# AlexanderDzhoganov/sphereflake-raytracer

Hardware: AMD Instinct MI355X
Metric: Mrays/sec into G-buffer at 1920x1080 depth-8; frame time ms (higher is better)
Workload: dtype f32

## Files before the change

### __graft_entry__.py

```python
import os
import subprocess
import sys

REPO = os.path.dirname(os.path.abspath(__file__))
PKG = os.path.join(REPO, "sphereflake-raytracer_amd")


def _paths():
    for p in (REPO, PKG):
        if p not in sys.path:
            sys.path.insert(0, p)


def build() -> None:
    _paths()
    jobs = str(min(16, os.cpu_count() or 1))
    subprocess.check_call(["make", "-s", "-j", jobs, "-C", PKG, "all"])
    subprocess.check_call(["make", "-s", "-C", PKG, "testlibs"])
    subprocess.check_call(["make", "-s", "-C", os.path.join(REPO, "oracle"), "all"])
    if os.path.isdir("/root/reference/sphereflake"):
        subprocess.check_call(["make", "-s", "-C", os.path.join(REPO, "oracle"), "ref"])
    import sphereflake_amd
    sphereflake_amd.lib()


def smoke() -> None:
    _paths()
    import numpy as np
    import sphereflake_amd as sf
    from oracle import pyoracle
    if not os.path.exists(sf.LIB_PATH):
        sf.build()
    W, H, K = 96, 64, 0.25
    with sf.Sphereflake(W, H, device=0) as s:
        cam = sf.config_camera(W, H, K)
        s.SetCamera(cam)
        s.Render(emit_aux=True)
        pos, nrm, mint, idx = s.download(aux=True)
        st = s.stats()
    o, tl, tr, bl = cam.corners()
    setup = {"W": W, "H": H, "origin": o, "tl": tl, "tr": tr, "bl": bl,
             "root": sf.root_transform(o), "children": sf.child_transforms()}
    ref = pyoracle.render(setup)
    for k, got in (("pos4", pos), ("nrm4", nrm), ("minT", mint), ("index", idx)):
        if not np.array_equal(np.ascontiguousarray(ref[k]).view(np.uint8), np.ascontiguousarray(got).view(np.uint8)):
            raise AssertionError(f"smoke: {k} differs from the oracle")
    if st.max_depth != ref["stats"]["max_depth"]:
        raise AssertionError("smoke: max depth differs from the oracle")
    print(f"smoke ok: {W}x{H} K={K} max_depth={st.max_depth} hits={ref['stats']['hits']}")


if __name__ == "__main__":
    build()
    if len(sys.argv) > 1 and sys.argv[1] == "smoke":
        smoke()
```

### sphereflake-raytracer_amd/csrc/sf_internal.h

```cpp
#pragma once

#include <stdint.h>

#if defined(__HIPCC__) || defined(__HIP__)
#define SF_HD __host__ __device__
#else
#define SF_HD
#endif

#define SF_DEPTH_TABLE 33
#ifndef SF_OCCL_MARGIN
#define SF_OCCL_MARGIN 0x1.8p-9f
#endif
#define SF_TILE 8
#define SF_WAVES_PER_BLOCK 4
#ifndef SF_WAVES_PER_EU
#define SF_WAVES_PER_EU 8
#endif
#ifndef SF_PAIR_WAVES_PER_EU
#define SF_PAIR_WAVES_PER_EU 7
#endif
#ifndef SF_TRACE_WAVES
#define SF_TRACE_WAVES 1
#endif
#define SF_LDS_ROOT 16
#define SF_LDS_CONE 8
#define SF_LDS_PLANE 38
#define SF_LDS_COLS 27
#define SF_LDS_TABLE (SF_LDS_PLANE + 3 * SF_LDS_COLS)
#define SF_LDS_E 32
#define SF_LDS_LEVEL (SF_LDS_TABLE + SF_LDS_E + 1)
#define SF_LDS_WAVE_FLOATS(levels) (SF_LDS_ROOT + SF_LDS_CONE + ((levels) - 1) * SF_LDS_LEVEL)
#define SF_RAYS_CSTACK (3 * 64)
#define SF_LDS_RAYS_FLOATS(levels) (SF_LDS_WAVE_FLOATS((levels) + 1) + (levels) * SF_RAYS_CSTACK)

#define SF_QUEUES 32u
#define SF_QUEUE_STRIDE 32u
#define SF_QUEUE_WORD(parity, k) (SF_QUEUE_STRIDE + ((parity) * SF_QUEUES + (k)) * SF_QUEUE_STRIDE)
#define SF_COUNTER_WORDS (SF_QUEUE_STRIDE + 2u * SF_QUEUES * SF_QUEUE_STRIDE)

#define SF_DIAG_SLOTS 16
#define SF_DIAG_WAVES 65536u
#define SF_TRACE_WORDS(ntiles) ((size_t)(ntiles) * 15u + SF_DIAG_SLOTS + 2u * SF_DIAG_WAVES)

#define SF_FLAG_NO_LOD_CULL 1u
#define SF_FLAG_NO_CONE_CULL 2u
#define SF_FLAG_DIAG_HALF 4u
#define SF_FLAG_DIAG_HALF_SEL 8u
#define SF_FLAG_DIAG_UNITS 0x20u
#define SF_FLAG_DIAG_NO_OWNER 0x40u
#define SF_FLAG_PRIO_FLAT 0x80u
#define SF_FLAG_NO_OCCL_CULL 0x100u
#define SF_FLAG_NO_DEPTH_SEED 0x10u
#define SF_FLAG_NO_FRONT_FIRST 0x200u
#define SF_FLAG_DIAG_FORCE_RETRACE 0x400u
#define SF_FLAG_TIE_INLINE 0x800u
#define SF_FLAG_REDO_PASS 0x1000u
#define SF_FLAG_SUBTREE 0x2000u
#define SF_FLAG_HALVES 0x4000u
#define SF_FLAG_FORCE_MIXED 0x8000u

struct DepthTables {
    float r2_bound[SF_DEPTH_TABLE];
    float r2_self[SF_DEPTH_TABLE];
    float scale[SF_DEPTH_TABLE];
    float lod[SF_DEPTH_TABLE];
};

struct DeviceConsts {
    float child[9][16];
    DepthTables dt;
    float depth8[SF_DEPTH_TABLE][8];
    uint32_t lut[2048];
    uint32_t sobol[2][52];
    float rw, rh;
    uint32_t fast_div, tx_magic;
};

struct PacketLane {
    float px, py, pz, nx, ny, nz, min_t;
    uint32_t pixel;
};

struct FrameArgs {
    uint32_t W, H;
    float fw, fh;
    float o[3], tl[3], dh[3], dv[3];
    float root[12];
    uint32_t tiles_x;
    uint32_t tile_rows;
    uint32_t tiles_per_band;
    uint32_t band_count, band_index;
    uint32_t compact;
    uint32_t packed;
    uint32_t max_depth;
    uint32_t emit_aux;
    uint32_t flags;
    const DeviceConsts* consts;
    float* pos;
    float* nrm;
    float* min_t;
    uint32_t* hit_index;
    int32_t* stats;
    uint64_t* tile_trace;
    uint64_t* phase_sums;
    uint32_t* counters;
    uint32_t* overflow_list;
    uint32_t parity;
    uint32_t* tile_cost;
    const uint32_t* tile_order;
    const uint32_t* order_meta;
    uint32_t* chunk_cnt;
    uint32_t* part_cost;
// ... 126 lines not shown
```

### sphereflake-raytracer_amd/csrc/sf_kernels.hip

```cpp
#include <hip/hip_runtime.h>
#include <float.h>
#include <stddef.h>
#include <stdint.h>

#include "sf_internal.h"

#pragma clang fp contract(off)

#define SF_MAX_LEVELS 31

namespace {

__device__ __forceinline__ float rsqrtps_x86(float x, const uint32_t* __restrict__ lut)
{
    const uint32_t b = __float_as_uint(x);
    const uint32_t E = (b >> 23) & 0xffu;
    const uint32_t key = ((E & 1u) << 10) | ((b & 0x7fffffu) >> 13);
    const int32_t E0 = (E & 1u) ? 127 : 128;
    const int32_t k = ((int32_t)E - E0) / 2;
    uint32_t r = (uint32_t)((int32_t)lut[key] - k * (1 << 23));
    if ((b & 0x7fffffffu) > 0x7f800000u) r = b | 0x00400000u;
    else if (E == 0u) r = (b & 0x80000000u) | 0x7f800000u;
    else if (b & 0x80000000u) r = 0xffc00000u;
    else if (E == 0xffu) r = 0u;
// ... 195 lines not shown
{
    __builtin_amdgcn_wave_barrier();
    __asm__ volatile("" ::: "memory");
}

__device__ __forceinline__ float readlane_f(float v, uint32_t l)
{
    return __int_as_float(__builtin_amdgcn_readlane(__float_as_int(v), (int)l));
}
__device__ __forceinline__ uint32_t writelane_u(uint32_t v, uint32_t l, uint32_t old)
{
    return (threadIdx.x & 63u) == l ? v : old;
}

__device__ int sf_amdgcn_writelane(int v, int l, int old) __asm("llvm.amdgcn.writelane.i32");
__device__ __forceinline__ uint32_t writelane_s(uint32_t v, uint32_t l, uint32_t old)
{
    return (uint32_t)sf_amdgcn_writelane((int)v, (int)l, (int)old);
}

__device__ __forceinline__ void wave_atomic_add_u64(uint64_t* p, uint64_t v)
{
    uint64_t saved;
    const uint32_t zero = 0u;
    __asm__ volatile(
        "s_mov_b64 %0, exec\n\t"
        "s_mov_b64 exec, 1\n\t"
        "global_atomic_add_x2 %1, %2, %3\n\t"
        "s_waitcnt vmcnt(0)\n\t"
        "s_mov_b64 exec, %0\n\t"
        : "=&s"(saved)
        : "v"(zero), "v"(v), "s"(p)
        : "memory");
}

#ifdef SF_PHASE_STAMPS
#define SF_STAMP_DECL uint64_t ph_last = __builtin_amdgcn_s_memtime(), ph_sum[7] = {0, 0, 0, 0, 0, 0, 0}
#define SF_STAMP(k)                                                                            \
    do {                                                                                       \
        uint64_t t_;                                                                           \
        __builtin_amdgcn_sched_barrier(0);                                                     \
        __asm__ volatile("s_memtime %0\n\ts_waitcnt lgkmcnt(0)" : "=s"(t_)::"memory");         \
        __builtin_amdgcn_sched_barrier(0);                                                     \
        ph_sum[k] += t_ - ph_last;                                                             \
        ph_last = t_;                                                                          \
    } while (0)
#define SF_STAMP_FLUSH(p)                                                                      \
    do {                                                                                       \
        if (p) {                                                                               \
            for (int k_ = 0; k_ < 7; ++k_) wave_atomic_add_u64((uint64_t*)(p) + k_, ph_sum[k_]);  \
        }                                                                                      \
    } while (0)
#elif defined(SF_COUNTS)
#define SF_STAMP_DECL uint64_t ph_sum[16] = {0, 0, 0, 0, 0, 0, 0, 0, 0, 0, 0, 0, 0, 0, 0, 0}
#define SF_STAMP(k)
#define SF_COUNT(k, v) (ph_sum[k] += (v))
#define SF_STAMP_FLUSH(p)                                                                      \
    do {                                                                                       \
        if (p) {                                                                               \
            ph_sum[15] = 1;                                                                    \
            for (int k_ = 0; k_ < 16; ++k_) wave_atomic_add_u64((uint64_t*)(p) + k_, ph_sum[k_]); \
        }                                                                                      \
    } while (0)
#else
#define SF_STAMP_DECL
#define SF_STAMP(k)
#define SF_STAMP_FLUSH(p) (void)(p)
#endif
#ifndef SF_COUNT
#define SF_COUNT(k, v)
#endif

__device__ __forceinline__ float4 depth_consts(const DeviceConsts* K, uint32_t d)
{
#if defined(__HIP_DEVICE_COMPILE__)
    typedef const __attribute__((address_space(4))) float4* ConstF4;
    typedef const __attribute__((address_space(4))) char* ConstC;
    return *(ConstF4)((ConstC)(const void*)K->depth8 + (d << 5));
#else
    return reinterpret_cast<const float4*>(K->depth8)[2u * d];
#endif
}
__device__ __forceinline__ float4 depth_consts_at(const DeviceConsts* K, uint32_t o)
{
#if defined(__HIP_DEVICE_COMPILE__)
    typedef const __attribute__((address_space(4))) float4* ConstF4;
    typedef const __attribute__((address_space(4))) char* ConstC;
    return *(ConstF4)((ConstC)(const void*)K->depth8 + o);
#else
    return reinterpret_cast<const float4*>(K->depth8)[o >> 4];
#endif
}
__device__ __forceinline__ float depth_word_at(const DeviceConsts* K, uint32_t o, uint32_t w)
{
#if defined(__HIP_DEVICE_COMPILE__)
    typedef const __attribute__((address_space(4))) float* ConstF;
    typedef const __attribute__((address_space(4))) char* ConstC;
    return *(ConstF)((ConstC)(const void*)K->depth8 + o + 4u * w);
#else
    return reinterpret_cast<const float*>(K->depth8)[(o >> 2) + w];
#endif
}
__device__ __forceinline__ float depth_leaf(const DeviceConsts* K, uint32_t d)
{
#if defined(__HIP_DEVICE_COMPILE__)
    typedef const __attribute__((address_space(4))) float* ConstF;
    typedef const __attribute__((address_space(4))) char* ConstC;
    return *(ConstF)((ConstC)(const void*)K->depth8 + (d << 5) + 16u);
#else
    return reinterpret_cast<const float4*>(K->depth8)[2u * d + 1u].x;
#endif
}

#define SF_STATUS_OVERFLOW 1u
// ... 80 lines not shown
}
template <class S2m>
__device__ __forceinline__ void stage_cone(const TraverseLds& L, uint32_t lane, bool cone_cull, float ax, float ay,
                                           float az, S2m s2m)
{
    float cosT = 0.0f, sinT = 1.0f;
    if (cone_cull) {
        const float sm = __builtin_amdgcn_sqrtf(wave_max_pos(s2m())) * (1.0f + 0x1p-16f) + 0x1p-16f;
        if (sm < 0.5f) {
            sinT = sm;
            cosT = __builtin_amdgcn_sqrtf(1.0f - sm * sm) * (1.0f - 0x1p-16f);
        }
    }
    if (lane < 5u) L.cone()[lane] = lane == 0u ? ax : lane == 1u ? ay : lane == 2u ? az : lane == 3u ? cosT : sinT;
}

__device__ __forceinline__ uint64_t lod_expands(float tca, float d2, float xs, bool hb, uint64_t hbm, float R2b, float T,
                                                float Tfar)
{
    const uint64_t nearm = wave_ballot(tca < T);
    const uint64_t farm = wave_ballot(tca * (1.0f - 0x1p-8f) >= Tfar);
    if ((hbm & ~(nearm | farm)) == 0ull) return hbm & nearm;
    const float sq = __builtin_amdgcn_sqrtf(xs);
    const float s_lo = __uint_as_float((uint32_t)max((int32_t)__float_as_uint(sq) - 2, 0));
    const float s_hi = __uint_as_float(__float_as_uint(sq) + 2u);
    const float t_hi = tca - s_lo;
    const float t_lo = tca - s_hi;
    const uint64_t tinym = wave_ballot(xs < 0x1p-96f);
    const float thx = sel_mask(t_hi, __builtin_inff(), tinym);
    const float tlx = sel_mask(t_lo, -__builtin_inff(), tinym);
    const float th = hb ? thx : __builtin_inff();
    const float tl = hb ? tlx : __builtin_inff();
    uint64_t exm = wave_ballot(th < T);
    const uint64_t undm = wave_ballot(sel_mask(tl, __builtin_inff(), exm) < T);
    if (undm) {
        const float te = near_root_exact(tca, d2, R2b);
        exm |= undm & wave_ballot(te < T);
    }
    return exm;
}

__device__ __forceinline__ bool child_expands(float cx, float cy, float cz, float cc, float dx, float dy, float dz,
                                              float actv, float R2b, float T, float Tfar)
{
    const float tca = (cx * dx + cy * dy) + cz * dz;
    const float d2 = cc - tca * tca;
    const float xs = R2b - d2;
    const bool hb = __builtin_fminf(__builtin_fminf(tca, xs), actv) >= 0.0f;
    const uint64_t hbm = wave_ballot(hb);
    return hbm != 0ull && lod_expands(tca, d2, xs, hb, hbm, R2b, T, Tfar) != 0ull;
}

template <bool ANYHIT, bool INDEX_ORDER = false>
__device__ __forceinline__ uint64_t accept_self(HitState& h, uint64_t& ancm, uint32_t& status, bool flag_ties,
                                                const float4 pc, float tca, float d2, uint32_t dd, float actv,
                                                uint32_t idx, float R2s)
{
    const uint64_t hsm = wave_ballot(__builtin_fminf(__builtin_fminf(tca, R2s - d2), actv) >= 0.0f);
    if (hsm) {
        const float xs = R2s - d2;
        float ts;
        if ((wave_ballot(!(xs >= 0x1p-96f)) & hsm) != 0ull) ts = near_root_exact(tca, d2, R2s);
        else ts = near_root_big(tca, xs);
        uint64_t accm = hsm & wave_ballot(ts < h.minT);
        if constexpr (ANYHIT) {
            uint32_t hd = (uint32_t)h.depth;
            sel_in_place(hd, dd, accm);
            h.depth = (int32_t)hd;
            return accm;
        }
        const uint64_t tie = hsm & wave_ballot(ts == h.minT);
        if constexpr (INDEX_ORDER) accm |= tie & ancm;
        else if (tie != 0ull) {
            accm |= tie & ancm;
            if (flag_ties && (tie & ~ancm) != 0ull) status |= SF_STATUS_TIE;
        }
        sel_in_place(h.minT, ts, accm);
        sel_in_place(h.cx, pc.x, accm);
        sel_in_place(h.cy, pc.y, accm);
        sel_in_place(h.cz, pc.z, accm);
        sel_in_place(h.index, idx, accm);
        uint32_t hd = (uint32_t)h.depth;
        sel_in_place(hd, dd, accm);
        h.depth = (int32_t)hd;
        ancm |= accm;
        return accm;
    }
    return 0ull;
}

template <bool ANYHIT>
__device__ __forceinline__ uint64_t occluded(float tca, float minT, float cull_t, float cull_r)
{
    float v = tca - minT;
    if constexpr (!ANYHIT) v = __builtin_fminf(v, tca - cull_t);
    return wave_ballot(v - SF_OCCL_MARGIN * tca > cull_r);
}

struct ChildBuild {
    float x, y, z, w;
    uint32_t M, front;
    float4 dtc;
};
__device__ __forceinline__ ChildBuild build_children(const DeviceConsts* K, const TraverseLds& L, const BuildLane& B,
                                                     const float4 pc, const float* col, uint32_t cs, uint32_t ko,
                                                     float kp, uint32_t index_order)
{
    lds_fence();
    const float3 p0 = *reinterpret_cast<const float3*>(col);
    const float3 p1 = *reinterpret_cast<const float3*>(col + cs);
    const float3 p2 = *reinterpret_cast<const float3*>(col + 2u * cs);
    const float4 cn = *reinterpret_cast<const float4*>(L.cone());
    const float sinT = L.cone()[4];
    const float4 dtn = depth_consts_at(K, ko - (1u << 5));
    const float4 dtc = depth_consts_at(K, ko);
    const float sm = B.bc == 3u ? dtn.z : 1.0f;
    const float b0 = B.b0 * sm, b1 = B.b1 * sm, b2 = B.b2 * sm;
    const float x = __builtin_fmaf(pc.x, B.b3, (p0.x * b0 + p1.x * b1) + p2.x * b2);
    const float y = __builtin_fmaf(pc.y, B.b3, (p0.y * b0 + p1.y * b1) + p2.y * b2);
    const float z = __builtin_fmaf(pc.z, B.b3, (p0.z * b0 + p1.z * b1) + p2.z * b2);
    const float w = (x * x + y * y) + z * z;
    const float R2b = dtc.x;
    const float ax = cn.x, ay = cn.y, az = cn.z, cosT = cn.w;
    const float ca = __builtin_fmaf(x, ax, __builtin_fmaf(y, ay, z * az));
    const float sq = __builtin_amdgcn_sqrtf(__builtin_fmaxf(__builtin_fmaf(-ca, ca, w), 0.0f));
    const float X = __builtin_fmaf(sq, cosT, -(ca * sinT));
    const float Y = __builtin_fmaf(X, X, -(R2b + w * (0x1p-18f + 0x1p-19f)));
    const float reg = __builtin_fmaf(w, 1.0f - 0x1p-16f, -2.0f * R2b);
    const float mk = __builtin_fminf(__builtin_fminf(ca, reg), __builtin_fminf(X, Y));
    uint32_t M = (uint32_t)(wave_ballot(!(mk > 0.0f)) >> 32) & 0x1ffu;
    M = __builtin_amdgcn_readfirstlane(M);
    const uint32_t front = ((uint32_t)(wave_ballot(ca < kp) >> 32) & 0x1ffu) | index_order;
    return ChildBuild{ x, y, z, w, M, front, dtc };
}

template <int PW>
__device__ __forceinline__ void traverse_packet(const DeviceConsts* __restrict__ K, const float* root,
                                                float* __restrict__ Lbase, const float4 bcol, uint32_t levels, float dx,
                                                float dy, float dz, bool valid, HitState& h, int32_t& maxd,
                                                uint32_t& status, uint32_t K_flags)
{
    const uint32_t lane = threadIdx.x & 63u;
    const TraverseLds L{ Lbase };
    const bool cone_cull = (K_flags & SF_FLAG_NO_CONE_CULL) == 0u;
    SF_STAMP_DECL;

    reset_hit(h, FLT_MAX);
    uint64_t ancm = 0ull;

    const float rcx = root[9], rcy = root[10], rcz = root[11];
    const float rcc = (rcx * rcx + rcy * rcy) + rcz * rcz;
    bool ex0;
    {
        const float4 dt0 = depth_consts(K, 0u);
        const float tca = (rcx * dx + rcy * dy) + rcz * dz;
        const float d2 = rcc - tca * tca;
        const bool hb = valid && group_any<PW>(tca >= 0.0f) && group_any<PW>(d2 <= dt0.x);
        ex0 = hb && group_any<PW>(near_root(tca, d2, dt0.x) < dt0.w);
    }
    if (!wave_ballot(ex0)) return;
    maxd = 0;

    {
        const float ax = readlane_f(dx, 36u), ay = readlane_f(dy, 36u), az = readlane_f(dz, 36u);
        stage_cone(L, lane, cone_cull, ax, ay, az, [&] { return cone_s2m(dx, dy, dz, ax, ay, az); });
    }

    const uint32_t bi = build_child(lane);
    const uint32_t bc = lane < 27u ? lane / 9u : 3u;
    const bool lod_cull = (K_flags & SF_FLAG_NO_LOD_CULL) == 0u;
    auto leaf_front = [&](const float4 pc, float R2b) -> bool {
        const float tca = (pc.x * dx + pc.y * dy) + pc.z * dz;
        return wave_ballot(!(tca >= 0.0f && tca * tca >= R2b * (1.0f + 0x1p-6f))) == 0ull;
    };
    const float b[4] = { bcol.x, bcol.y, bcol.z, bcol.w };
    const uint32_t slot = bc == 3u ? bi * 4u : SF_LDS_PLANE + bc * SF_LDS_COLS + bi * 3u;

    uint32_t d = 0;
    uint32_t idxB = 1;

    auto self_test = [&](const float4 pc, uint32_t dd, uint64_t actm, uint32_t idx, float R2s) {
        const float tca = (pc.x * dx + pc.y * dy) + pc.z * dz;
        const float d2 = pc.w - tca * tca;
        const bool f0 = tca >= 0.0f, in = d2 <= R2s;
        const uint64_t hsm = actm & wave_ballot(group_any<PW>(f0) && group_any<PW>(in));
        if (hsm) {
            const float xs = R2s - d2;
            float ts;
// ... 148 lines not shown
        lds_fence();
        {
            const uint32_t pc = __builtin_amdgcn_readlane(stk_pc, d);
            pend = pc & 0x1ffu;
            leafN = pc >> 9;
            idxB = (uint32_t)__builtin_amdgcn_readlane(stk_ix, d);
        }
        eN = L.E(d)[lane];
        (void)__builtin_amdgcn_readfirstlane(eN);
        SF_STAMP(5);
    }
    h.hit = h.depth >= 0;
}

struct DepthSeed {
    int32_t own = -1;
    int32_t word = -1;
    __device__ __forceinline__ int32_t depth(uint32_t flags) const
    {
        int32_t seed = -1;
        if ((flags & (SF_FLAG_NO_OCCL_CULL | SF_FLAG_NO_DEPTH_SEED)) == 0u) {
            const int32_t w = __builtin_amdgcn_readfirstlane(word);
            const int32_t o = __builtin_amdgcn_readfirstlane(own);
            const int32_t m = o > w ? o : w;
            seed = (m > 0 ? m : 0) & 31;
        }
        return __builtin_amdgcn_readfirstlane(seed);
    }
};
__device__ __forceinline__ int32_t stats_word(const FrameArgs& a)
{
    return __hip_atomic_load(&a.stats[0], __ATOMIC_RELAXED, __HIP_MEMORY_SCOPE_AGENT);
}

__device__ __forceinline__ uint32_t split_mask(uint32_t q, uint32_t idxB)
{
    const uint32_t m9 = (0x111u << ((q - idxB) & 3u)) & 0x1ffu;
    return m9 | (m9 << 16);
}

template <bool COMPACT = false, bool SPLIT = false, bool SHADOW = false>
__device__ __forceinline__ void traverse_ray(const DeviceConsts* __restrict__ K, const float* root, float* __restrict__ Lbase,
                                             const float4 bcol, uint32_t levels, float dx, float dy, float dz, bool valid,
                                             HitState& h, int32_t& maxd, uint32_t& status, uint32_t K_flags,
                                             uint64_t* phase_sums = nullptr, uint32_t axl = 36u,
                                             uint64_t* tile_counts = nullptr, uint32_t split_q = 0u,
                                             uint32_t split_depth = 0u, int32_t seed = -1, float bound = FLT_MAX)
{
    const uint32_t lane = threadIdx.x & 63u;
    const TraverseLds L{ Lbase };
    const bool cone_cull = (K_flags & SF_FLAG_NO_CONE_CULL) == 0u;
    const bool occl_cull = (K_flags & SF_FLAG_NO_OCCL_CULL) == 0u;
    const bool front_first = (K_flags & (SF_FLAG_NO_OCCL_CULL | SF_FLAG_NO_FRONT_FIRST)) == 0u;
    SF_STAMP_DECL;

    reset_hit(h, SHADOW ? bound : FLT_MAX);
    uint64_t ancm = 0ull;

    const float rcx = root[9], rcy = root[10], rcz = root[11];
    const float rcc = (rcx * rcx + rcy * rcy) + rcz * rcz;
    uint64_t ex0m;
    {
        const float4 dt0 = depth_consts(K, 0u);
        const float tca = (rcx * dx + rcy * dy) + rcz * dz;
        const float d2 = rcc - tca * tca;
        const bool hb = valid && tca >= 0.0f && d2 <= dt0.x;
        const uint64_t hbm = wave_ballot(hb);
        if (hbm == 0ull) return;
        ex0m = lod_expands(tca, d2, dt0.x - d2, hb, hbm, dt0.x, dt0.w, depth_word_at(K, 0u, 6u));
        if (ex0m == 0ull) return;
    }
    maxd = 0;

    {
        const float ax = readlane_f(dx, axl), ay = readlane_f(dy, axl), az = readlane_f(dz, axl);
        stage_cone(L, lane, cone_cull, ax, ay, az, [&] { return cone_s2m(dx, dy, dz, ax, ay, az); });
    }

    float cull_t = depth_consts(K, (uint32_t)(seed > 0 ? seed : 0) + 1u).w;

    const BuildLane B = build_lane(bcol, lane, build_child(lane));

    uint32_t d = 0;
    uint32_t idxB = 1;

    auto self_test = [&](const float4 pc, float tca, float d2, uint32_t dd, float actv, uint32_t idx,
                         float R2s) -> uint64_t {
        return accept_self<SHADOW>(h, ancm, status, front_first, pc, tca, d2, dd, actv, idx, R2s);
    };

    const uint32_t lv32 = __builtin_amdgcn_readfirstlane(levels << 5);
    const uint32_t index_order = front_first ? 0u : 0x1ffu;
    auto expand = [&](const float4 pc, const float* col, uint32_t cs, uint32_t d, float actv,
                      float* tb, uint32_t ko, float kp) -> uint32_t {
        d = __builtin_amdgcn_readfirstlane(d);
        SF_COUNT(0, 1);
        SF_COUNT(7, __builtin_popcountll(wave_ballot(actv >= 0.0f)));
        const ChildBuild cb = build_children(K, L, B, pc, col, cs, ko, kp, index_order);
        if (ko < lv32) {
            *reinterpret_cast<float3*>(tb + B.slot) = make_float3(cb.x, cb.y, cb.z);
            *(B.bc == 3u ? tb + B.slot + 3u : L.cone() + 5u) = cb.w;
            return (cb.M & cb.front) | ((cb.M & ~cb.front) << 16);
        }
        {
            const float R2b = cb.dtc.x, T = cb.dtc.w, Tfar = depth_word_at(K, ko, 6u);
            uint32_t M = cb.M;
            while (M) {
                const uint32_t i = __builtin_ctz(M);
                M &= ~(1u << i);
                const float cx = readlane_f(cb.x, 32u + i), cy = readlane_f(cb.y, 32u + i);
                const float cz = readlane_f(cb.z, 32u + i), cc = readlane_f(cb.w, 32u + i);
                if (child_expands(cx, cy, cz, cc, dx, dy, dz, actv, R2b, T, Tfar)) {
                    status |= SF_STATUS_OVERFLOW;
                    break;
                }
            }
            return 0u;
        }
    };

    uint32_t stk_pc = 0u, stk_ix = 0u;
    float* tcur = L.table(0u);
    uint32_t kofs = 1u << 5;
    float R2c = depth_consts_at(K, kofs).x;
    uint32_t C = 0u;
    float actv;
    uint32_t actbits;
    {
        lds_fence();
        const float4 pc = *reinterpret_cast<const float4*>(L.root());
        actv = sel_mask(-1.0f, __builtin_inff(), ex0m);
        actbits = 0u;
        sel_in_place(actbits, 1u, ex0m);
        const float tca = (pc.x * dx + pc.y * dy) + pc.z * dz;
        const float d2 = pc.w - tca * tca;
        const uint64_t acc0 = self_test(pc, tca, d2, 0u, actv, 0u, depth_consts(K, 0u).y);
        bool live = true;
        if constexpr (SHADOW) {
            actv = sel_mask(actv, -1.0f, acc0);
            sel_in_place(actbits, 0u, acc0);
            live = wave_ballot(actbits != 0u) != 0ull;
        }
        if (live && !__builtin_amdgcn_readfirstlane((int)(pc.w > depth_leaf(K, 0u))))
            C = expand(pc, L.root() + 4u, 4u, 0u, actv, tcur, kofs, readlane_f(tca, axl));
        else SF_COUNT(4, 1);
        if constexpr (SPLIT) {
            if (split_depth == 1u) C &= split_mask(split_q, 1u);
        }
    }

    for (;;) {
        d = __builtin_amdgcn_readfirstlane(d);
        SF_STAMP(0);
        if (C) {
            const uint32_t p = __builtin_ctz(C);
            __asm__("s_bitset0_b32 %0, %1" : "+s"(C) : "s"(p));
// ... 9 lines not shown
            SF_COUNT(1, 1);
#ifdef SF_COUNTS
            {
                const uint32_t na = __builtin_popcountll(wave_ballot(actv >= 0.0f));
                SF_COUNT(5, na);
                SF_COUNT(6, __builtin_popcountll(hbm));
                SF_COUNT(10, d >= 4u ? 1 : 0);
                SF_COUNT(11, d >= 4u ? na : 0);
                SF_COUNT(14, na <= 32u ? 1 : 0);
            }
#endif
            if (hbm == 0ull) {
                SF_COUNT(2, 1);
                continue;
            }
            const float4 dk = depth_consts_at(K, kofs + 16u);
            const float Tfar = dk.z;
            const float cull_r = dk.y;
            const uint64_t exm = lod_expands(tca, d2, xs, hb, hbm, dc.x, dc.w, Tfar);
            SF_STAMP(2);
            if (exm == 0ull) continue;
            SF_COUNT(3, 1);
            if (!SHADOW && (int32_t)d + 1 > maxd) {
                maxd = (int32_t)d + 1;
                if ((int32_t)d + 1 > seed) cull_t = depth_consts_at(K, kofs + (1u << 5)).w;
            }
            uint64_t amx = exm;
            if (occl_cull) {
                amx = exm & ~occluded<SHADOW>(tca, h.minT, cull_t, cull_r);
                SF_COUNT(13, 1);
                SF_COUNT(12, amx == 0ull ? 1 : 0);
                if (amx == 0ull) continue;
            }
            float avx = sel_mask(-1.0f, __builtin_inff(), amx);
            const uint64_t acc = self_test(pc, tca, d2, d + 1u, avx, idxB + c, dc.y);
            SF_STAMP(4);
            if constexpr (SHADOW) {
                if (acc != 0ull) {
                    amx &= ~acc;
                    avx = sel_mask(avx, -1.0f, acc);
                    actv = sel_mask(actv, -1.0f, acc);
                    sel_in_place(actbits, 0u, acc);
                    if (wave_ballot(actbits != 0u) == 0ull) break;
                    if (amx == 0ull) continue;
                }
            }
            if (wave_ballot(pc.w > dk.x) != 0ull) {
                SF_COUNT(4, 1);
                SF_COUNT(8, 1);
                SF_COUNT(9, __builtin_popcountll(amx));
                ancm &= wave_ballot(h.depth != (int32_t)d + 1);
                continue;
            }
            stk_pc = writelane_s(C, d, stk_pc);
            stk_ix = writelane_s(idxB, d, stk_ix);
            {
                const uint32_t bit = 2u << d;
                uint32_t ab = actbits & ~bit;
                sel_in_place(ab, ab | bit, amx);
                actbits = ab;
            }
            idxB = 9u * (idxB + c) + 1u;
            d += 1u;
            actv = avx;
            SF_STAMP(1);
            const float* const col = tcur + SF_LDS_PLANE + 3u * c;
            tcur += SF_LDS_LEVEL;
            kofs += 1u << 5;
            C = expand(pc, col, SF_LDS_COLS, d, avx, tcur, kofs, readlane_f(tca, axl));
            if constexpr (SPLIT) {
                if (d + 1u == split_depth) C &= split_mask(split_q, idxB);
            }
            R2c = depth_consts_at(K, kofs).x;
            if (COMPACT && C != 0u) {
                __builtin_amdgcn_sched_barrier(0);
                const uint64_t actm = wave_ballot(avx > 0.0f);
                const uint32_t na = (uint32_t)__builtin_popcountll(actm);
                const uint32_t M = (C | (C >> 16)) & 0x1ffu;
                if (na <= 7u && __builtin_popcount(M) >= 3) {
                    const float R2b = depth_consts(K, d + 1u).x;
                    const uint32_t rank = __builtin_amdgcn_mbcnt_hi((uint32_t)(actm >> 32),
                                                                    __builtin_amdgcn_mbcnt_lo((uint32_t)actm, 0u));
                    float* const sc = reinterpret_cast<float*>(L.E(d)) + 1;
                    *reinterpret_cast<float4*>(sc + (avx > 0.0f ? 4u * rank : 28u)) = make_float4(dx, dy, dz, 0.0f);
                    lds_fence();
                    uint32_t ln = lane;
                    __asm__ volatile("" : "+v"(ln));
                    const uint32_t g = (ln * 37u) >> 8;
                    const uint32_t sl = ln - 7u * g;
                    const float4 q = *reinterpret_cast<const float4*>(sc + 4u * sl);
                    const bool ok = sl < na && g < 9u && ((M >> g) & 1u) != 0u;
                    const uint32_t gi = g < 9u ? g : 8u;
                    const float4 cg = *reinterpret_cast<const float4*>(L.table(d) + gi * 4u);
                    const float tca = (cg.x * q.x + cg.y * q.y) + cg.z * q.z;
                    const float d2 = cg.w - tca * tca;
                    const float xs = R2b - d2;
                    const uint64_t bal =
                        wave_ballot(__builtin_fminf(__builtin_fminf(tca, xs), ok ? __builtin_inff() : -1.0f) >= 0.0f);
                    const uint32_t kk = ln < 9u ? ln : 0u;
                    const uint64_t grp = (bal >> (7u * kk)) & 0x7full;
                    const uint32_t hitm = (uint32_t)wave_ballot(ln < 9u && grp != 0ull) & 0x1ffu;
                    const uint32_t keep = __builtin_amdgcn_readfirstlane(hitm);
                    C &= keep | (keep << 16);
                }
            }
            SF_STAMP(6);
            continue;
        }
        ancm &= wave_ballot(h.depth != (int32_t)d);
        if (d == 0u) break;
        d -= 1u;
        tcur -= SF_LDS_LEVEL;
        kofs -= 1u << 5;
        R2c = depth_consts_at(K, kofs).x;
        {
            const uint32_t pw = __builtin_amdgcn_readlane(stk_pc, d);
            C = pw;
            idxB = (uint32_t)__builtin_amdgcn_readlane(stk_ix, d);
        }
        actv = ((actbits >> d) & 1u) ? __builtin_inff() : -1.0f;
        SF_STAMP(5);
    }
// ... 1833 lines not shown
template <RootStage STAGE, bool STATS, class GroupFn>
__device__ __forceinline__ void fixup_groups(const FrameArgs a, float* lds, const uint32_t* overflow_list,
                                             uint32_t* counters, uint32_t parity, GroupFn group_fn)
{
    const uint32_t n = counters[parity];
    if (blockIdx.x == 0 && threadIdx.x == 0) {
        counters[parity ^ 1u] = 0u;
        counters[2] += n;
    }
    if (blockIdx.x >= n) return;
    int32_t maxd = -1;
    float closest = FLT_MAX;
    uint32_t unresolved = 0u;
    if constexpr (STAGE == RootStage::Once) stage_root(lds, a.root);
    const float4 bcol = build_column(a.consts);
    for (uint32_t i = blockIdx.x; i < n; i += gridDim.x) {
        if constexpr (STAGE == RootStage::PerGroup) {
            lds_fence();
            stage_root(lds, a.root);
        }
        if constexpr (STATS) {
            const TileStats st = group_fn(overflow_list[i], bcol);
            maxd = st.maxd > maxd ? st.maxd : maxd;
            closest = fminf(closest, st.closest);
            unresolved += st.overflowed ? 1u : 0u;
        } else {
            group_fn(overflow_list[i], bcol);
        }
    }
    if constexpr (STATS) publish_stats(a, maxd, closest, unresolved);
}

template <bool FIXUP>
__device__ __forceinline__ TileStats trace_dir_group(const FrameArgs& a, const float* __restrict__ dirs, uint32_t stride,
                                                     float* __restrict__ L, const float4 bcol, uint32_t group,
                                                     uint32_t levels, uint32_t* overflow_list, uint32_t* overflow_count)
{
    const DeviceConsts* __restrict__ K = a.consts;
    const GroupLane g = group_lane(a, group);
    const float* const dp = dirs + (size_t)g.ray * stride;
    float dx = dp[0], dy = dp[1], dz = dp[2];
    normalize3(dx, dy, dz, K->lut);
    const bool fin = finite3(dx, dy, dz);
    const uint64_t finm = wave_ballot(fin);
    HitState h = miss_state();
    int32_t maxd = -1;
    uint32_t status = 0u;
    if (finm != 0ull) {
        const uint32_t axl = axis_lane(finm, g.mid);
        const float ax = readlane_f(dx, axl), ay = readlane_f(dy, axl), az = readlane_f(dz, axl);
        dx = fin ? dx : ax;
        dy = fin ? dy : ay;
        dz = fin ? dz : az;
        const uint32_t flags = (a.flags & (SF_FLAG_NO_CONE_CULL | SF_FLAG_NO_OCCL_CULL | SF_FLAG_NO_FRONT_FIRST)) |
                               (FIXUP ? SF_FLAG_NO_FRONT_FIRST : 0u);
        traverse_ray<>(K, a.root, L, bcol, levels, dx, dy, dz, g.valid && fin, h, maxd, status, flags, nullptr, axl);
    }
    const bool flagged = status != 0u;
    if (!FIXUP && flagged) flag_group(overflow_list, overflow_count, group);
    if (g.valid) store_ray(a, g.ray, dx, dy, dz, h, K->lut);
    return group_stats(maxd, g.valid ? h.minT : FLT_MAX, flagged);
}

}

extern "C" __global__ __launch_bounds__(64) void sf_trace_dirs_wave(FrameArgs a, const float* dirs, uint32_t stride,
                                                                    uint32_t groups, uint32_t* overflow_list,
                                                                    uint32_t* overflow_count)
{
    extern __shared__ float lds[];
    if (blockIdx.x >= groups) return;
    stage_root(lds, a.root);
    const TileStats st = trace_dir_group<false>(a, dirs, stride, lds, build_column(a.consts), blockIdx.x, a.max_depth,
                                                overflow_list, overflow_count);
    publish_stats(a, st.maxd, st.closest, 0u);
}

extern "C" __global__ __launch_bounds__(64) void sf_trace_dirs_fixup(FrameArgs a, const float* dirs, uint32_t stride,
                                                                     const uint32_t* overflow_list, uint32_t* counters,
                                                                     uint32_t parity)
{
    extern __shared__ float lds[];
    fixup_groups<RootStage::Once, true>(a, lds, overflow_list, counters, parity,
                                        [&](uint32_t group, const float4 bcol) {
        return trace_dir_group<true>(a, dirs, stride, lds, bcol, group, SF_MAX_LEVELS, nullptr, nullptr);
    });
}

namespace {

#define SF_STATUS_ZSIGN 4u

template <bool ANYHIT = false>
__device__ __forceinline__ void traverse_mixed(const DeviceConsts* __restrict__ K, float* __restrict__ Lbase,
                                               float* __restrict__ cstk, const float4 bcol, uint32_t levels, float dx,
                                               float dy, float dz, float ocx, float ocy, float ocz, bool valid,
                                               HitState& h, int32_t& maxd, uint32_t& status, uint32_t K_flags,
                                               float bound = FLT_MAX)
{
    const uint32_t lane = threadIdx.x & 63u;
    const TraverseLds L{ Lbase };
    const bool occl_cull = (K_flags & SF_FLAG_NO_OCCL_CULL) == 0u;

    reset_hit(h, ANYHIT ? bound : FLT_MAX);
    uint64_t ancm = 0ull;

    const float occ0 = (ocx * ocx + ocy * ocy) + ocz * ocz;
// ... 126 lines not shown
            const float* const col = tcur + SF_LDS_PLANE + 3u * c;
            tcur += SF_LDS_LEVEL;
            kofs += 1u << 5;
            expand(col, SF_LDS_COLS, tcur, kofs);
            R2c = depth_consts_at(K, kofs).x;
            C = 0x1ffu;
            continue;
        }
        ancm &= wave_ballot(h.depth != (int32_t)d);
        if (d == 0u) break;
        d -= 1u;
        tcur -= SF_LDS_LEVEL;
        kofs -= 1u << 5;
        R2c = depth_consts_at(K, kofs).x;
        C = (uint32_t)__builtin_amdgcn_readlane(stk_pc, d);
        idxB = (uint32_t)__builtin_amdgcn_readlane(stk_ix, d);
        actv = ((actbits >> d) & 1u) ? __builtin_inff() : -1.0f;
        const float* const cl = cs + d * SF_RAYS_CSTACK;
        ocx = cl[0];
        ocy = cl[64];
        ocz = cl[128];
    }
    h.hit = h.depth >= 0;
}

template <bool FIXUP, bool ONE = false>
__device__ __forceinline__ TileStats trace_ray_group(const FrameArgs& a, const float* __restrict__ origins,
                                                     const float* __restrict__ dirs, uint32_t ostride, uint32_t dstride,
                                                     uint32_t rpo, uint32_t mixed_ok, float* __restrict__ L,
                                                     const float4 bcol, uint32_t group, uint32_t levels,
                                                     uint32_t* overflow_list, uint32_t* overflow_count)
{
    const DeviceConsts* __restrict__ K = a.consts;
    const uint32_t lane = threadIdx.x & 63u;
    const GroupLane g = group_lane(a, group);
    const uint32_t ray = g.ray, mid = g.mid;
    const bool valid = g.valid;
    const float* const dp = dirs + (size_t)ray * dstride;
    const float* const op = origins + (size_t)(rpo > 1u ? ray / rpo : ray) * ostride;
    float dx = dp[0], dy = dp[1], dz = dp[2];
    const float rx = 0.0f - op[0], ry = 0.0f - op[1], rz = 0.0f - op[2];
    normalize3(dx, dy, dz, K->lut);
    const bool on = valid && finite3(dx, dy, dz);
    const uint64_t onm = wave_ballot(on);
    HitState h = miss_state();
    int32_t maxd = -1;
    uint32_t status = 0u;
    if (onm != 0ull) {
        const uint32_t f0 = __builtin_amdgcn_readfirstlane((uint32_t)__builtin_ctzll(onm));
        const bool same = __float_as_uint(rx) == __float_as_uint(readlane_f(rx, f0)) &&
                          __float_as_uint(ry) == __float_as_uint(readlane_f(ry, f0)) &&
                          __float_as_uint(rz) == __float_as_uint(readlane_f(rz, f0));
        const bool mixed = !ONE && ((onm & ~wave_ballot(same)) != 0ull || (a.flags & SF_FLAG_FORCE_MIXED) != 0u);
        const uint32_t culls = a.flags & (SF_FLAG_NO_CONE_CULL | SF_FLAG_NO_OCCL_CULL | SF_FLAG_NO_FRONT_FIRST);
        uint64_t todo = onm;
        if (!ONE && mixed && mixed_ok != 0u) {
            float* const cstk = L + SF_LDS_WAVE_FLOATS(levels + 1u);
            traverse_mixed(K, L, cstk, bcol, levels, dx, dy, dz, rx, ry, rz, on, h, maxd, status, culls);
            if (status & SF_STATUS_ZSIGN) {
                status = 0u;
                maxd = -1;
                h = miss_state();
            } else {
                todo = 0ull;
            }
        }
        while (todo != 0ull) {
            const uint32_t l0 = __builtin_amdgcn_readfirstlane((uint32_t)__builtin_ctzll(todo));
            float r[12];
#pragma unroll
            for (int k = 0; k < 9; ++k) r[k] = a.root[k];
            r[9] = readlane_f(rx, l0);
            r[10] = readlane_f(ry, l0);
            r[11] = readlane_f(rz, l0);
            const bool mine = on && (ONE || (__float_as_uint(rx) == __float_as_uint(r[9]) &&
                                             __float_as_uint(ry) == __float_as_uint(r[10]) &&
                                             __float_as_uint(rz) == __float_as_uint(r[11])));
            const uint64_t m = todo & wave_ballot(mine);
            const bool member = ((m >> lane) & 1ull) != 0ull;
            const uint32_t axl = axis_lane(m, mid, l0);
            const float ax = readlane_f(dx, axl), ay = readlane_f(dy, axl), az = readlane_f(dz, axl);
            lds_fence();
            stage_root(L, r);
            HitState h1;
            int32_t md = -1;
            uint32_t st = 0u;
            traverse_ray<>(K, r, L, bcol, levels, member ? dx : ax, member ? dy : ay, member ? dz : az, member, h1, md,
                           st, culls | (FIXUP ? SF_FLAG_NO_FRONT_FIRST : 0u), nullptr, axl);
            if (member) h = h1;
            maxd = md > maxd ? md : maxd;
            status |= st;
            todo &= ~m;
            if (ONE) break;
        }
    }
    const bool flagged = status != 0u;
    if (!FIXUP && flagged) flag_group(overflow_list, overflow_count, group);
    if (valid) store_ray(a, ray, dx, dy, dz, h, K->lut);
    return group_stats(maxd, valid ? h.minT : FLT_MAX, flagged);
}

}

extern "C" __global__ __launch_bounds__(64) void sf_trace_rays_wave(FrameArgs a, const float* origins, const float* dirs,
                                                                    uint32_t ostride, uint32_t dstride, uint32_t rpo,
                                                                    uint32_t mixed_ok, uint32_t groups,
                                                                    uint32_t* overflow_list, uint32_t* overflow_count)
// ... 828 lines not shown
```

### sphereflake-raytracer_amd/sphereflake_amd/__init__.py

```python
from __future__ import annotations

import ctypes
import os
import subprocess
import threading
from dataclasses import dataclass

import numpy as np

PKG_DIR = os.path.dirname(os.path.abspath(__file__))
ROOT_DIR = os.path.dirname(PKG_DIR)
LIB_PATH = os.environ.get("SF_LIB") or os.path.join(ROOT_DIR, "build", "libsphereflake_hip.so")
HEADER_PATH = os.path.join(os.path.dirname(ROOT_DIR), "include", "sphereflake", "sf.h")

SF_OK, SF_EINVAL, SF_ENOMEM, SF_EHIP, SF_ENODEV, SF_ENOVIEW, SF_EDEPTH, SF_ESTATE = 0, -1, -2, -3, -4, -5, -6, -7
SF_KERNEL_WAVE, SF_KERNEL_PER_RAY = 0, 1
SF_MAX_DEPTH_LIMIT = 31
FLT_MAX = float(np.finfo(np.float32).max)

DEFAULT_CAMERA_POSITION = (-5.4098, -7.2139, 1.19006)
DEFAULT_PITCH = -1.371
DEFAULT_YAW = 0.921999
SF_DIAG_WAVES = 65536


class SphereflakeError(RuntimeError):
    def __init__(self, code: int, what: str = ""):
        self.code = code
        msg = _strerror(code)
        super().__init__(f"{what}: {msg} ({code})" if what else f"{msg} ({code})")


class sf_render_params(ctypes.Structure):
    _fields_ = [("band_rows", ctypes.c_uint32), ("band_count", ctypes.c_uint32),
                ("band_index", ctypes.c_uint32), ("compact", ctypes.c_uint32),
                ("kernel", ctypes.c_uint32), ("emit_aux", ctypes.c_uint32),
                ("max_depth", ctypes.c_uint32), ("packed", ctypes.c_uint32),
                ("stream", ctypes.c_void_p)]


class sf_dirs_params(ctypes.Structure):
    _fields_ = [("width", ctypes.c_uint32), ("height", ctypes.c_uint32), ("stride", ctypes.c_uint32),
                ("max_depth", ctypes.c_uint32), ("stream", ctypes.c_void_p)]


class sf_rays_params(ctypes.Structure):
    _fields_ = [("width", ctypes.c_uint32), ("height", ctypes.c_uint32), ("dir_stride", ctypes.c_uint32),
                ("origin_stride", ctypes.c_uint32), ("rays_per_origin", ctypes.c_uint32),
                ("max_depth", ctypes.c_uint32), ("stream", ctypes.c_void_p)]


class sf_shadow_params(ctypes.Structure):
    _fields_ = [("light", ctypes.c_float * 3), ("bias", ctypes.c_float), ("origin", ctypes.c_float * 3),
                ("use_origin", ctypes.c_uint32), ("width", ctypes.c_uint32), ("height", ctypes.c_uint32),
                ("max_depth", ctypes.c_uint32), ("stream", ctypes.c_void_p)]


SF_SHADOW_LIGHTS_MAX = 64


class sf_shadows_params(ctypes.Structure):
    _fields_ = [("lights", ctypes.POINTER(ctypes.c_float)), ("weights", ctypes.POINTER(ctypes.c_float)),
                ("n", ctypes.c_uint32), ("bias", ctypes.c_float), ("origin", ctypes.c_float * 3),
                ("use_origin", ctypes.c_uint32), ("width", ctypes.c_uint32), ("height", ctypes.c_uint32),
                ("max_depth", ctypes.c_uint32), ("stream", ctypes.c_void_p)]


class sf_sun_params(ctypes.Structure):
    _fields_ = [("dir", ctypes.c_float * 3), ("distance", ctypes.c_float), ("bias", ctypes.c_float),
                ("origin", ctypes.c_float * 3), ("use_origin", ctypes.c_uint32), ("width", ctypes.c_uint32),
                ("height", ctypes.c_uint32), ("max_depth", ctypes.c_uint32), ("stream", ctypes.c_void_p)]


class sf_stats(ctypes.Structure):
    _fields_ = [("max_depth", ctypes.c_int32), ("closest", ctypes.c_float),
                ("rays", ctypes.c_int64), ("overflow_tiles", ctypes.c_int64)]
# ... 873 lines not shown
        with self._mutex:
            _check(lib().sf_download_async(self._ctx, vp(g.positions), vp(g.normals), None, None,
                                           ctypes.c_void_p(stream) if stream else None), "download_async", self._ctx)

    def post_params(self, **kw) -> sf_post_params:
        p = sf_post_params()
        _check(lib().sf_post_defaults(self._ctx, ctypes.byref(p)), "sf_post_defaults")
        for k, v in kw.items():
            if k == "camera_position":
                p.camera_position[:] = [float(x) for x in _f32(v, 3)]
            elif k == "stream":
                p.stream = v
            else:
                setattr(p, k, v)
        return p

    def PostProcess(self, pos_ptr: int = 0, nrm_ptr: int = 0, rgba_ptr: int = 0, ao_ptr: int = 0, **kw):
        p = self.post_params(**kw)
        vp = lambda x: ctypes.c_void_p(x) if x else None
        with self._mutex:
            _check(lib().sf_post_process(self._ctx, ctypes.byref(p), vp(pos_ptr), vp(nrm_ptr), vp(rgba_ptr),
                                         vp(ao_ptr)), "sf_post_process", self._ctx)

    def download_image(self) -> np.ndarray:
        img = np.empty((self.height, self.width, 4), np.uint8)
        with self._mutex:
            _check(lib().sf_download_image(self._ctx, img.ctypes.data_as(ctypes.c_void_p)), "sf_download_image",
                   self._ctx)
        return img

    @staticmethod
    def ssao_noise() -> np.ndarray:
        out = np.empty((64 * 64, 4), np.float32)
        _check(lib().sf_ssao_noise(_fp(out)), "sf_ssao_noise")
        return out

    def save_image(self, path: str, what: int = SF_DUMP_NORMALS) -> None:
        with self._mutex:
            _check(lib().sf_save_image(self._ctx, os.fsencode(path), int(what)), "sf_save_image", self._ctx)

    @staticmethod
    def save_ppm(path: str, rgb) -> None:
        a = np.clip(np.asarray(rgb, np.float32), 0.0, 1.0)
        b = (a * 255.0 + 0.5).astype(np.uint8)
        with open(path, "wb") as f:
            f.write(f"P6 {b.shape[1]} {b.shape[0]} 255\n".encode())
            f.write(np.ascontiguousarray(b[:, :, :3]).tobytes())

    def tile_trace(self, enable: bool | None = None):
        if enable is not None:
            _check(lib().sf_set_tile_trace(self._ctx, int(bool(enable))), "sf_set_tile_trace", self._ctx)
            return None
        n = ((self.width + 7) // 8) * ((self.height + 7) // 8)
        out = np.zeros(15 * n + 16 + 2 * SF_DIAG_WAVES, np.uint64)
        _check(lib().sf_get_tile_trace(self._ctx, out.ctypes.data_as(ctypes.POINTER(ctypes.c_uint64)), out.size),
               "sf_get_tile_trace", self._ctx)
        self.phase_sums = out[3 * n:3 * n + 16]
        self.unit_trace = out[3 * n + 16:15 * n + 16].reshape(4 * n, 3)
        self.wave_trace = out[15 * n + 16:].reshape(SF_DIAG_WAVES, 2)
        return out[:3 * n].reshape(n, 3)

    def tile_order(self):
        n = ((self.width + 7) // 8) * ((self.height + 7) // 8)
        order = np.zeros(4 * n, np.uint32)
        cost = np.zeros(n, np.uint32)
        P = ctypes.POINTER(ctypes.c_uint32)
        k = lib().sf_get_tile_order(self._ctx, order.ctypes.data_as(P), cost.ctypes.data_as(P), 4 * n)
        if k < 0:
            _check(k, "sf_get_tile_order", self._ctx)
        return (order[:k], cost[:int(lib().sf_order_units(self._ctx))]) if k else None

    def kernel_timing(self, enable: bool | None = None, n: int = 64, period: int = 1):
        if enable is not None:
            k = max(1, int(period)) if enable else 0
            _check(lib().sf_set_kernel_timing(self._ctx, k), "sf_set_kernel_timing", self._ctx)
            return None
        out = np.zeros(n, np.float32)
        k = lib().sf_kernel_times(self._ctx, out.ctypes.data_as(_F), n)
        if k < 0:
            _check(k, "sf_kernel_times", self._ctx)
        return out[:k]

    def kernel_clocks(self, n: int = 64):
        out = np.zeros(n, np.float32)
        k = lib().sf_kernel_clocks(self._ctx, out.ctypes.data_as(_F), n)
        if k < 0:
            _check(k, "sf_kernel_clocks", self._ctx)
        return out[:k]

    def stats(self) -> sf_stats:
        self._raise_worker_error()
        s = sf_stats()
        with self._mutex:
            _check(lib().sf_get_stats(self._ctx, ctypes.byref(s)), "sf_get_stats", self._ctx)
        return s

    def lean_launches(self) -> int:
        return int(lib().sf_lean_launches(self._ctx))

    def pair_launches(self) -> int:
        return int(lib().sf_pair_launches(self._ctx))

    def GetMaxDepthReached(self) -> int:
        return int(self.stats().max_depth)

    def ResetMaxDepthReached(self):
        _check(lib().sf_reset_max_depth(self._ctx), "ResetMaxDepthReached")

    def GetRaysPerSecond(self) -> int:
        return int(self.stats().rays)

    def ResetRaysPerSecond(self):
# ... 269 lines not shown
```

Baseline: 41190.

## Intersect all-leaf child sets inline instead of pushing a traversal level

When every child produced by an expansion is a leaf (beyond the LOD bound at the next depth), the wave tests those children directly in a flat loop rather than pushing the stack and descending another level. The aim is to cut stack writes, LDS table builds and loop overhead at the deepest traversal level. It adds a ballot plus a depth-constant load per expansion and more register pressure in the main traversal kernel. A flag can disable the path, and a new counter slot tracks how often it is taken.

```diff
diff --git a/__graft_entry__.py b/__graft_entry__.py
--- a/__graft_entry__.py
+++ b/__graft_entry__.py
@@ -17,6 +17,7 @@
     jobs = str(min(16, os.cpu_count() or 1))
     subprocess.check_call(["make", "-s", "-j", jobs, "-C", PKG, "all"])
     subprocess.check_call(["make", "-s", "-C", PKG, "testlibs"])
+    subprocess.check_call(["make", "-s", "-j", jobs, "-C", PKG, "COUNTS=1", "build_counts/libsphereflake_hip.so"])
     subprocess.check_call(["make", "-s", "-C", os.path.join(REPO, "oracle"), "all"])
     if os.path.isdir("/root/reference/sphereflake"):
         subprocess.check_call(["make", "-s", "-C", os.path.join(REPO, "oracle"), "ref"])
diff --git a/sphereflake-raytracer_amd/csrc/sf_internal.h b/sphereflake-raytracer_amd/csrc/sf_internal.h
--- a/sphereflake-raytracer_amd/csrc/sf_internal.h
+++ b/sphereflake-raytracer_amd/csrc/sf_internal.h
@@ -39,7 +39,7 @@
 #define SF_QUEUE_WORD(parity, k) (SF_QUEUE_STRIDE + ((parity) * SF_QUEUES + (k)) * SF_QUEUE_STRIDE)
 #define SF_COUNTER_WORDS (SF_QUEUE_STRIDE + 2u * SF_QUEUES * SF_QUEUE_STRIDE)
 
-#define SF_DIAG_SLOTS 16
+#define SF_DIAG_SLOTS 17
 #define SF_DIAG_WAVES 65536u
 #define SF_TRACE_WORDS(ntiles) ((size_t)(ntiles) * 15u + SF_DIAG_SLOTS + 2u * SF_DIAG_WAVES)
 
@@ -59,6 +59,7 @@
 #define SF_FLAG_SUBTREE 0x2000u
 #define SF_FLAG_HALVES 0x4000u
 #define SF_FLAG_FORCE_MIXED 0x8000u
+#define SF_FLAG_NO_LEAF_LOOP 0x10000u
 
 struct DepthTables {
     float r2_bound[SF_DEPTH_TABLE];
diff --git a/sphereflake-raytracer_amd/csrc/sf_kernels.hip b/sphereflake-raytracer_amd/csrc/sf_kernels.hip
--- a/sphereflake-raytracer_amd/csrc/sf_kernels.hip
+++ b/sphereflake-raytracer_amd/csrc/sf_kernels.hip
@@ -271,14 +271,14 @@
         }                                                                                      \
     } while (0)
 #elif defined(SF_COUNTS)
-#define SF_STAMP_DECL uint64_t ph_sum[16] = {0, 0, 0, 0, 0, 0, 0, 0, 0, 0, 0, 0, 0, 0, 0, 0}
+#define SF_STAMP_DECL uint64_t ph_sum[SF_DIAG_SLOTS] = {0, 0, 0, 0, 0, 0, 0, 0, 0, 0, 0, 0, 0, 0, 0, 0, 0}
 #define SF_STAMP(k)
 #define SF_COUNT(k, v) (ph_sum[k] += (v))
 #define SF_STAMP_FLUSH(p)                                                                      \
     do {                                                                                       \
         if (p) {                                                                               \
             ph_sum[15] = 1;                                                                    \
-            for (int k_ = 0; k_ < 16; ++k_) wave_atomic_add_u64((uint64_t*)(p) + k_, ph_sum[k_]); \
+            for (int k_ = 0; k_ < SF_DIAG_SLOTS; ++k_) wave_atomic_add_u64((uint64_t*)(p) + k_, ph_sum[k_]); \
         }                                                                                      \
     } while (0)
 #else
@@ -465,40 +465,45 @@
 }
 
 template <bool ANYHIT, bool INDEX_ORDER = false>
+__device__ __forceinline__ uint64_t accept_hits(HitState& h, uint64_t& ancm, uint32_t& status, bool flag_ties,
+                                                const float4 pc, float tca, float d2, uint32_t dd, uint64_t hsm,
+                                                uint32_t idx, float R2s)
+{
+    const float xs = R2s - d2;
+    float ts;
+    if ((wave_ballot(!(xs >= 0x1p-96f)) & hsm) != 0ull) ts = near_root_exact(tca, d2, R2s);
+    else ts = near_root_big(tca, xs);
+    uint64_t accm = hsm & wave_ballot(ts < h.minT);
+    if constexpr (ANYHIT) {
+        uint32_t hd = (uint32_t)h.depth;
+        sel_in_place(hd, dd, accm);
+        h.depth = (int32_t)hd;
+        return accm;
+    }
+    const uint64_t tie = hsm & wave_ballot(ts == h.minT);
+    if constexpr (INDEX_ORDER) accm |= tie & ancm;
+    else if (tie != 0ull) {
+        accm |= tie & ancm;
+        if (flag_ties && (tie & ~ancm) != 0ull) status |= SF_STATUS_TIE;
+    }
+    sel_in_place(h.minT, ts, accm);
+    sel_in_place(h.cx, pc.x, accm);
+    sel_in_place(h.cy, pc.y, accm);
+    sel_in_place(h.cz, pc.z, accm);
+    sel_in_place(h.index, idx, accm);
+    uint32_t hd = (uint32_t)h.depth;
+    sel_in_place(hd, dd, accm);
+    h.depth = (int32_t)hd;
+    ancm |= accm;
+    return accm;
+}
+template <bool ANYHIT, bool INDEX_ORDER = false>
 __device__ __forceinline__ uint64_t accept_self(HitState& h, uint64_t& ancm, uint32_t& status, bool flag_ties,
                                                 const float4 pc, float tca, float d2, uint32_t dd, float actv,
                                                 uint32_t idx, float R2s)
 {
     const uint64_t hsm = wave_ballot(__builtin_fminf(__builtin_fminf(tca, R2s - d2), actv) >= 0.0f);
-    if (hsm) {
-        const float xs = R2s - d2;
-        float ts;
-        if ((wave_ballot(!(xs >= 0x1p-96f)) & hsm) != 0ull) ts = near_root_exact(tca, d2, R2s);
-        else ts = near_root_big(tca, xs);
-        uint64_t accm = hsm & wave_ballot(ts < h.minT);
-        if constexpr (ANYHIT) {
-            uint32_t hd = (uint32_t)h.depth;
-            sel_in_place(hd, dd, accm);
-            h.depth = (int32_t)hd;
-            return accm;
-        }
-        const uint64_t tie = hsm & wave_ballot(ts == h.minT);
-        if constexpr (INDEX_ORDER) accm |= tie & ancm;
-        else if (tie != 0ull) {
-            accm |= tie & ancm;
-            if (flag_ties && (tie & ~ancm) != 0ull) status |= SF_STATUS_TIE;
-        }
-        sel_in_place(h.minT, ts, accm);
-        sel_in_place(h.cx, pc.x, accm);
-        sel_in_place(h.cy, pc.y, accm);
-        sel_in_place(h.cz, pc.z, accm);
-        sel_in_place(h.index, idx, accm);
-        uint32_t hd = (uint32_t)h.depth;
-        sel_in_place(hd, dd, accm);
-        h.depth = (int32_t)hd;
-        ancm |= accm;
-        return accm;
-    }
+    if (hsm) return accept_hits<ANYHIT, INDEX_ORDER>(h, ancm, status, flag_ties, pc, tca, d2, dd, hsm, idx, R2s);
     return 0ull;
 }
 
@@ -547,6 +552,44 @@
     return ChildBuild{ x, y, z, w, M, front, dtc };
 }
 
+struct LeafNode {
+    float w;
+    uint32_t M;
+    float4 dc, dk;
+};
+__device__ __forceinline__ bool all_leaves(const DeviceConsts* K, LeafNode& ln, uint32_t ko)
+{
+    ln.dk = depth_consts_at(K, ko + 16u);
+    const uint32_t leafm = (uint32_t)(wave_ballot(ln.w > ln.dk.x) >> 32);
+    return __builtin_amdgcn_readfirstlane(ln.M & ~leafm) == 0u;
+}
+__device__ __forceinline__ void leaf_children(HitState& h, uint64_t& ancm, uint32_t& status, bool flag_ties, bool occl_cull,
+                                              float dx, float dy, float dz, float actv, uint32_t C, const float* tb,
+                                              const float4 dc, const float4 dk, float cull_t, uint32_t dd, uint32_t idxB)
+{
+    const float R2b = dc.x, R2s = dc.y, T = dc.w, cull_r = dk.y, Tfar = dk.z;
+    lds_fence();
+    while (C) {
+        const uint32_t p = __builtin_ctz(C);
+        __asm__("s_bitset0_b32 %0, %1" : "+s"(C) : "s"(p));
+        const uint32_t c = p & 15u;
+        const float4 pc = *reinterpret_cast<const float4*>(tb + c * 4u);
+        const float tca = (pc.x * dx + pc.y * dy) + pc.z * dz;
+        const float d2 = pc.w - tca * tca;
+        const bool hs = __builtin_fminf(__builtin_fminf(tca, R2s - d2), actv) >= 0.0f;
+        const uint64_t hsm = wave_ballot(hs);
+        if (hsm == 0ull) continue;
+        uint64_t amx = lod_expands(tca, d2, R2b - d2, hs, hsm, R2b, T, Tfar);
+        if (amx == 0ull) continue;
+        if (occl_cull) {
+            amx &= ~occluded<false>(tca, h.minT, cull_t, cull_r);
+            if (amx == 0ull) continue;
+        }
+        accept_hits<false>(h, ancm, status, flag_ties, pc, tca, d2, dd, amx, idxB + c, R2s);
+        ancm &= wave_ballot(h.depth != (int32_t)dd);
+    }
+}
+
 template <int PW>
 __device__ __forceinline__ void traverse_packet(const DeviceConsts* __restrict__ K, const float* root,
                                                 float* __restrict__ Lbase, const float4 bcol, uint32_t levels, float dx,
@@ -801,6 +844,8 @@
     const bool cone_cull = (K_flags & SF_FLAG_NO_CONE_CULL) == 0u;
     const bool occl_cull = (K_flags & SF_FLAG_NO_OCCL_CULL) == 0u;
     const bool front_first = (K_flags & (SF_FLAG_NO_OCCL_CULL | SF_FLAG_NO_FRONT_FIRST)) == 0u;
+    constexpr bool LEAF = !COMPACT && !SPLIT && !SHADOW;
+    const bool leaf_loop = LEAF && (K_flags & SF_FLAG_NO_LEAF_LOOP) == 0u;
     SF_STAMP_DECL;
 
     reset_hit(h, SHADOW ? bound : FLT_MAX);
@@ -841,7 +886,7 @@
     const uint32_t lv32 = __builtin_amdgcn_readfirstlane(levels << 5);
     const uint32_t index_order = front_first ? 0u : 0x1ffu;
     auto expand = [&](const float4 pc, const float* col, uint32_t cs, uint32_t d, float actv,
-                      float* tb, uint32_t ko, float kp) -> uint32_t {
+                      float* tb, uint32_t ko, float kp, LeafNode* ln = nullptr) -> uint32_t {
         d = __builtin_amdgcn_readfirstlane(d);
         SF_COUNT(0, 1);
         SF_COUNT(7, __builtin_popcountll(wave_ballot(actv >= 0.0f)));
@@ -849,8 +894,10 @@
         if (ko < lv32) {
             *reinterpret_cast<float3*>(tb + B.slot) = make_float3(cb.x, cb.y, cb.z);
             *(B.bc == 3u ? tb + B.slot + 3u : L.cone() + 5u) = cb.w;
+            if (ln) *ln = LeafNode{ cb.w, cb.M, cb.dtc, cb.dtc };
             return (cb.M & cb.front) | ((cb.M & ~cb.front) << 16);
         }
+        if (ln) *ln = LeafNode{ cb.w, 0u, cb.dtc, cb.dtc };
         {
             const float R2b = cb.dtc.x, T = cb.dtc.w, Tfar = depth_word_at(K, ko, 6u);
             uint32_t M = cb.M;
@@ -966,6 +1013,21 @@
                 ancm &= wave_ballot(h.depth != (int32_t)d + 1);
                 continue;
             }
+            uint32_t Cn = 0u;
+            if constexpr (LEAF) {
+                const float* const col = tcur + SF_LDS_PLANE + 3u * c;
+                LeafNode ln;
+                Cn = expand(pc, col, SF_LDS_COLS, d + 1u, avx, tcur + SF_LDS_LEVEL, kofs + (1u << 5),
+                            readlane_f(tca, axl), &ln);
+                if (leaf_loop && Cn != 0u && (int32_t)d + 2 <= (maxd > seed ? maxd : seed) &&
+                    all_leaves(K, ln, kofs + (1u << 5))) {
+                    SF_COUNT(16, 1);
+                    leaf_children(h, ancm, status, front_first, occl_cull, dx, dy, dz, avx, Cn, tcur + SF_LDS_LEVEL,
+                                  ln.dc, ln.dk, cull_t, d + 2u, 9u * (idxB + c) + 1u);
+                    ancm &= wave_ballot(h.depth != (int32_t)d + 1);
+                    continue;
+                }
+            }
             stk_pc = writelane_s(C, d, stk_pc);
             stk_ix = writelane_s(idxB, d, stk_ix);
             {
@@ -978,10 +1040,16 @@
             d += 1u;
             actv = avx;
             SF_STAMP(1);
-            const float* const col = tcur + SF_LDS_PLANE + 3u * c;
-            tcur += SF_LDS_LEVEL;
-            kofs += 1u << 5;
-            C = expand(pc, col, SF_LDS_COLS, d, avx, tcur, kofs, readlane_f(tca, axl));
+            if constexpr (LEAF) {
+                tcur += SF_LDS_LEVEL;
+                kofs += 1u << 5;
+                C = Cn;
+            } else {
+                const float* const col = tcur + SF_LDS_PLANE + 3u * c;
+                tcur += SF_LDS_LEVEL;
+                kofs += 1u << 5;
+                C = expand(pc, col, SF_LDS_COLS, d, avx, tcur, kofs, readlane_f(tca, axl));
+            }
             if constexpr (SPLIT) {
                 if (d + 1u == split_depth) C &= split_mask(split_q, idxB);
             }
@@ -2921,7 +2989,8 @@
         dx = fin ? dx : ax;
         dy = fin ? dy : ay;
         dz = fin ? dz : az;
-        const uint32_t flags = (a.flags & (SF_FLAG_NO_CONE_CULL | SF_FLAG_NO_OCCL_CULL | SF_FLAG_NO_FRONT_FIRST)) |
+        const uint32_t flags = (a.flags & (SF_FLAG_NO_CONE_CULL | SF_FLAG_NO_OCCL_CULL | SF_FLAG_NO_FRONT_FIRST |
+                                           SF_FLAG_NO_LEAF_LOOP)) |
                                (FIXUP ? SF_FLAG_NO_FRONT_FIRST : 0u);
         traverse_ray<>(K, a.root, L, bcol, levels, dx, dy, dz, g.valid && fin, h, maxd, status, flags, nullptr, axl);
     }
@@ -3154,7 +3223,8 @@
                           __float_as_uint(ry) == __float_as_uint(readlane_f(ry, f0)) &&
                           __float_as_uint(rz) == __float_as_uint(readlane_f(rz, f0));
         const bool mixed = !ONE && ((onm & ~wave_ballot(same)) != 0ull || (a.flags & SF_FLAG_FORCE_MIXED) != 0u);
-        const uint32_t culls = a.flags & (SF_FLAG_NO_CONE_CULL | SF_FLAG_NO_OCCL_CULL | SF_FLAG_NO_FRONT_FIRST);
+        const uint32_t culls = a.flags & (SF_FLAG_NO_CONE_CULL | SF_FLAG_NO_OCCL_CULL | SF_FLAG_NO_FRONT_FIRST |
+                                          SF_FLAG_NO_LEAF_LOOP);
         uint64_t todo = onm;
         if (!ONE && mixed && mixed_ok != 0u) {
             float* const cstk = L + SF_LDS_WAVE_FLOATS(levels + 1u);
diff --git a/sphereflake-raytracer_amd/sphereflake_amd/__init__.py b/sphereflake-raytracer_amd/sphereflake_amd/__init__.py
--- a/sphereflake-raytracer_amd/sphereflake_amd/__init__.py
+++ b/sphereflake-raytracer_amd/sphereflake_amd/__init__.py
@@ -22,6 +22,7 @@
 DEFAULT_PITCH = -1.371
 DEFAULT_YAW = 0.921999
 SF_DIAG_WAVES = 65536
+SF_DIAG_SLOTS = 17
 
 
 class SphereflakeError(RuntimeError):
@@ -1001,12 +1002,13 @@
             _check(lib().sf_set_tile_trace(self._ctx, int(bool(enable))), "sf_set_tile_trace", self._ctx)
             return None
         n = ((self.width + 7) // 8) * ((self.height + 7) // 8)
-        out = np.zeros(15 * n + 16 + 2 * SF_DIAG_WAVES, np.uint64)
+        out = np.zeros(15 * n + SF_DIAG_SLOTS + 2 * SF_DIAG_WAVES, np.uint64)
         _check(lib().sf_get_tile_trace(self._ctx, out.ctypes.data_as(ctypes.POINTER(ctypes.c_uint64)), out.size),
                "sf_get_tile_trace", self._ctx)
-        self.phase_sums = out[3 * n:3 * n + 16]
-        self.unit_trace = out[3 * n + 16:15 * n + 16].reshape(4 * n, 3)
-        self.wave_trace = out[15 * n + 16:].reshape(SF_DIAG_WAVES, 2)
+        k = SF_DIAG_SLOTS
+        self.phase_sums = out[3 * n:3 * n + k]
+        self.unit_trace = out[3 * n + k:15 * n + k].reshape(4 * n, 3)
+        self.wave_trace = out[15 * n + k:].reshape(SF_DIAG_WAVES, 2)
         return out[:3 * n].reshape(n, 3)
 
     def tile_order(self):
```

Result: no change. 41160 (median of 2 runs) (-0.1%).
